# andrewcsmith/soundsym

Measured on AMD Instinct MI355X. Metric: segment-pairs/sec (DTW cost+argmin), higher is better.
Workload: dtype f32

## Files before the change

### soundsym_amd/csrc/dtw_filter.hip

```cpp
#include "ssym_internal.hpp"
#include "dtw_filter_kernel.hpp"
#include "dtw_filter_wg_kernel.hpp"
#include "dtw_filter_wg2_kernel.hpp"
#include "dtw_filter_pk_kernel.hpp"
#include "dtw_filter_sp_kernel.hpp"
#include "dtw_band_kernel.hpp"

#include <algorithm>
#include <atomic>
#include <cmath>
#include <cstdlib>

namespace ssym {

static std::atomic<unsigned long long> g_filter_wg_launches{0};
static std::atomic<unsigned long long> g_filter_wg2_launches{0};
static std::atomic<bool> g_filter_wg2{true};

int filter_pieces(int dim)
{
    static const bool k48 = ssym_knob("SSYM_FILTER_K48") != nullptr;
    return dim > kFilterMaxDim2 ? 1 : (k48 ? 2 : 3);
}

__global__ void build_filter_records_kernel(const double *__restrict__ raw, const uint64_t *__restrict__ off,
                                            const uint32_t *__restrict__ perm, uint32_t n, uint32_t dim,
                                            uint32_t dimUse, uint32_t frames_pad, int is_source,
                                            int lead, int pieces, double scale, _Float16 *__restrict__ rec,
                                            unsigned *__restrict__ resid)
{
    const uint32_t s = blockIdx.y;
    const uint32_t seg = perm[s];
    const uint32_t slot = blockIdx.x * blockDim.x + threadIdx.x;
    if (slot >= frames_pad)
        return;
    _Float16 out[kFilterRecHalfs];
#pragma unroll
    for (int i = 0; i < kFilterRecHalfs; ++i)
        out[i] = (_Float16)0.0f;
    const uint32_t nf = seg < n ? (uint32_t)(off[seg + 1] - off[seg]) : 0u;
    const uint32_t first = lead < 0 ? frames_pad - nf : (uint32_t)lead;
    const bool real = slot >= first && slot < first + nf;
    const uint32_t f = slot - first;
    const int nbase = pieces == 3 ? 28 : (pieces == 2 ? 3 : 1) * (int)dimUse;
    const int npieces = pieces == 3 ? 2 : 3;
    if (!real && is_source)
        out[filter_slot_offset(nbase)] = (_Float16)__builtin_inff();
    if (real) {
        const double *p = raw + (off[seg] + f) * dim;
        double nrm = 0.0, res2 = 0.0;
        for (uint32_t e = 0; e < dimUse; ++e) {
            const double v = p[e] * scale;
            const _Float16 h1 = (_Float16)v;
            const bool two = pieces == 2 || (pieces == 3 && (is_source || e < 2));
            const _Float16 h2 = two ? (_Float16)(v - (double)h1) : (_Float16)0.0f;
            const double vh = (double)h1 + (double)h2;
            nrm += vh * vh;
            res2 += (v - vh) * (v - vh);
            const _Float16 m1 = (_Float16)(-2.0f * (float)h1), m2 = (_Float16)(-2.0f * (float)h2);
            if (pieces == 2) {
                out[filter_slot_offset(3 * e + 0)] = is_source ? m1 : h1;
                out[filter_slot_offset(3 * e + 1)] = is_source ? m1 : h2;
                out[filter_slot_offset(3 * e + 2)] = is_source ? m2 : h1;
            } else if (pieces == 3) {
                out[filter_slot_offset(2 * e + 0)] = is_source ? m1 : h1;
                out[filter_slot_offset(2 * e + 1)] = is_source ? m2 : h1;
                if (e < 2)
                    out[filter_slot_offset(26 + e)] = is_source ? m1 : h2;
            } else {
                out[filter_slot_offset(e)] = is_source ? m1 : h1;
            }
        }
        const float r = __double2float_ru(sqrt(res2) / scale * 1.0000001);
        if (r > 0.0f)
            atomicMax(&resid[s], __float_as_uint(r));
        const _Float16 p1 = (_Float16)nrm;
        const _Float16 p2 = (_Float16)(nrm - (double)p1);
        const _Float16 p3 = (_Float16)(nrm - (double)p1 - (double)p2);
        const int mine = nbase + (is_source ? 0 : npieces), other = nbase + (is_source ? npieces : 0);
        out[filter_slot_offset(mine + 0)] = p1;
        out[filter_slot_offset(mine + 1)] = p2;
        out[filter_slot_offset(other + 0)] = (_Float16)1.0f;
        out[filter_slot_offset(other + 1)] = (_Float16)1.0f;
        if (npieces == 3) {
            out[filter_slot_offset(mine + 2)] = p3;
            out[filter_slot_offset(other + 2)] = (_Float16)1.0f;
        }
    }
    if (is_source) {
        _Float16 *dst = rec + ((size_t)s * frames_pad + slot) * kFilterRecHalfs;
#pragma unroll
        for (int i = 0; i < kFilterRecHalfs; ++i)
            dst[i] = out[i];
    } else {
#pragma unroll
        for (int h = 0; h < 2; ++h)
#pragma unroll
            for (int m = 0; m < kFilterKM; ++m) {
                _Float16 *dst = rec + tgt_rec_offset(s, frames_pad, slot, m, h);
#pragma unroll
                for (int i = 0; i < 8; ++i)
                    dst[i] = out[h * 24 + m * 8 + i];
            }
    }
}

static uint32_t band_slots(int radius, const SegmentSet &src, const SegmentSet &tgt)
{
    const uint32_t kb = (uint32_t)(2 * radius + 1 + 15) / 16 * 16;
    return std::max<uint32_t>(radius + src.max_frames, std::max<uint32_t>(tgt.max_frames, 1) + kb) + 1;
}
static size_t band_lds_bytes(int radius, const SegmentSet &src, const SegmentSet &tgt)
{
    return ((size_t)2 * band_slots(radius, src, tgt) * kFilterRecHalfs + kBandImagePad) * sizeof(_Float16);
}

bool filter_band_as_bound(const ssym_ctx *ctx, const SegmentSet &src, const SegmentSet &tgt)
{
    if (ctx->band < 0)
        return false;
    return 2 * ctx->band + 1 > 6 * 16 || band_lds_bytes(ctx->band, src, tgt) > 160 * 1024 - 64;
}

bool filter_supported(const ssym_ctx *ctx, const SegmentSet &src, const SegmentSet &tgt)
{
    if (src.light || tgt.light)
        return false;
    if (src.dim != tgt.dim)
        return false;
    if ((ctx->band < 0 || filter_band_as_bound(ctx, src, tgt)) && filter_shape((int)src.max_frames).nt == 0)
        return false;
    if (!std::isfinite(src.max_abs) || !std::isfinite(tgt.max_abs))
        return false;
    if (!std::isfinite(src.max_sqnorm_all) || !std::isfinite(tgt.max_sqnorm_all))
        return false;
    return src.n > 0 && tgt.n > 0;
}

static double common_scale(const SegmentSet &src, const SegmentSet &tgt)
{
    const double m = std::max(src.max_abs, tgt.max_abs);
    if (!(m > 0.0))
        return 1.0;
    int e = 0;
    (void)std::frexp(m, &e);
    e = std::min(std::max(6 - e, -100), 100);
    const double sq = std::max(src.max_sqnorm_all, tgt.max_sqnorm_all);
    while (e > -200 && sq * std::ldexp(1.0, 2 * e) * 1.01 >= 65000.0)
        --e;
    const double ideal = std::ldexp(1.0, e);
    if (src.rec && src.rec_scale > 0.0 && src.rec_scale <= ideal && src.rec_scale * 16.0 >= ideal)
        return src.rec_scale;
    return ideal;
}

static int32_t ensure_records(ssym_ctx *ctx, const SegmentSet &set, double scale, uint32_t slots, int lead)
{
    const size_t bytes = (size_t)set.n_pad * slots * kFilterRecHalfs * sizeof(_Float16);
    if (set.rec && set.rec_scale == scale && set.rec_bytes == bytes && set.rec_slots == slots &&
        set.rec_lead == lead)
        return SSYM_OK;
    if (set.rec && set.rec_bytes != bytes) {
        dev_free(ctx, set.rec);
        set.rec = nullptr;
    }
    if (!set.rec) {
        int32_t rca = dev_alloc(ctx, &set.rec, bytes);
        if (rca != SSYM_OK)
            return rca;
    }
    set.rec_bytes = bytes;
    dim3 grid((slots + 63) / 64, set.n_pad);
    const int dimUse = filter_dim_used((int)set.dim);
    unsigned *resid = (unsigned *)(set.max_sqnorm + 2 * (size_t)set.n_pad);
    SSYM_HIP_CHECK(ctx, hipMemsetAsync(resid, 0, sizeof(unsigned) * set.n_pad, ctx->stream));
    build_filter_records_kernel<<<grid, 64, 0, ctx->stream>>>(set.raw, set.off, set.perm, set.n, set.dim,
                                                              (uint32_t)dimUse, slots, set.is_source ? 1 : 0, lead,
                                                              filter_pieces(dimUse), scale,
                                                              (_Float16 *)set.rec, resid);
    SSYM_HIP_CHECK(ctx, hipGetLastError());
    set.rec_scale = scale;
    set.rec_slots = slots;
    set.rec_lead = lead;
    return SSYM_OK;
}

static FilterKnobs read_filter_knobs()
{
    FilterKnobs k;
    g_filter_wg2.store(true, std::memory_order_relaxed);
    if (!ssym_knob("SSYM_TEST_HOOKS"))
        return k;
    auto num = [](const char *name, int unset) {
        const char *v = ssym_knob(name);
        return v ? atoi(v) : unset;
    };
    k.pk = num("SSYM_FILTER_PK", 0) != 0;
    k.sp = num("SSYM_FILTER_SP", 1) != 0;
    const int mp = num("SSYM_SP_MULTIPAIR", 1);
    k.spMultipair = mp == 0 || mp == 2 ? mp : 1;
    k.spPairBlock = ssym_knob("SSYM_SP_PAIRBLOCK") ? std::max(num("SSYM_SP_PAIRBLOCK", 0), 0) : -1;
    k.wg = num("SSYM_FILTER_WG", k.wg) != 0;
    g_filter_wg2.store(num("SSYM_FILTER_WG2", 1) != 0, std::memory_order_relaxed);
    k.skip0 = num("SSYM_FILTER_SKIP0", 1) != 0;
    k.nt8 = ssym_knob("SSYM_FILTER_NT8") != nullptr;
    k.oneLaunch = ssym_knob("SSYM_FILTER_ONE_LAUNCH") != nullptr;
    k.longClasses = num("SSYM_FILTER_LONG_CLASSES", 1) != 0;
    k.pruneNt = num("SSYM_PRUNE_NT", 0);
    return k;
}

static const std::vector<uint32_t> &plan_lens(const SegmentSet &set, uint32_t group)
{
    if (set.plan_lens.size() != set.n_pad / group) {
        set.plan_lens.assign(set.n_pad / group, 0u);
        for (uint32_t slot = 0; slot < set.n; ++slot) {
            const uint32_t s = set.h_perm[slot];
            uint32_t &m = set.plan_lens[slot / group];
            m = std::max(m, (uint32_t)(set.h_off[s + 1] - set.h_off[s]));
        }
    }
    return set.plan_lens;
}

struct FilterCall {
    hipStream_t st;
    const SegmentSet &src, &tgt;
    bool sq;
    int ku;
    float outScale;
    float *handoff;
    unsigned *taskCtr;
    float *cmat;
    const float *abandon;
    unsigned long long *colCtr;
    const uint32_t *candSlot;
    bool wg2;
};

template <int NT, bool SQ, int KU>
static bool run_kernel(const FilterCall &c, const FilterLaunch &l)
{
    constexpr int OCC = NT == 1 ? 3 : NT == 8 ? 1 : 2;
    const dim3 grid(l.grid), block(64 * kFilterWavesPerBlock);
    const _Float16 *srec = (const _Float16 *)c.src.rec, *trec = (const _Float16 *)c.tgt.rec;
    const int rowsPad = (int)c.src.frames_pad, colsPad = (int)c.tgt.frames_pad, tgtPad = (int)c.tgt.n_pad;
    const int nSrcPairs = l.hi - l.lo, nTasks = nSrcPairs * (tgtPad / 32);
    unsigned *ctr = c.taskCtr + l.ctrSet * 8 * kTaskCtrStride;
    switch (l.kind) {
    case FilterKernel::Mp:
        if constexpr (NT == 1) {
            dtw_filter_sp_kernel<KU == 2 ? 3 : 2, SQ, 2, KU, kSpRowBlock, true><<<grid, block, 0, c.st>>>(
                srec, trec, c.src.len, c.tgt.len, rowsPad, colsPad, tgtPad, l.taskPairs, nSrcPairs, l.taskChunk, c.outScale,
                ctr, c.cmat, l.origin, l.lo, l.pairBlock);
            return true;
        }
        return false;
    case FilterKernel::Sp:
        if constexpr (NT <= 3 && (KU == 2 || NT <= 2)) {
            constexpr int OCCSP = (NT == 1 && KU == 2) ? 3 : (NT == 2 && KU == 2) ? SSYM_SP_OCC_NT2 : 2;
            dtw_filter_sp_kernel<NT, SQ, OCCSP, KU, kSpRowBlock><<<grid, block, 0, c.st>>>(
                srec, trec, c.src.len, c.tgt.len, rowsPad, colsPad, tgtPad, nSrcPairs, nTasks, l.taskChunk, c.outScale, ctr,
                c.cmat, l.origin, l.lo, l.pairBlock);
            return true;
        }
        return false;
    case FilterKernel::GenericSkip0:
        if constexpr (NT == 3 || NT == 4) {
            dtw_filter_kernel<NT, SQ, OCC, false, KU, true><<<grid, block, 0, c.st>>>(
                srec, trec, c.src.len, c.tgt.len, rowsPad, l.passes, colsPad, tgtPad, nSrcPairs, nTasks, l.taskChunk,
                c.outScale, c.handoff, ctr, c.cmat, nullptr, nullptr, nullptr, l.origin, l.lo);
            return true;
        }
        return false;
    case FilterKernel::Wg:
        if constexpr (NT == 4) {
            if (l.passes == 2 && c.wg2) {
                dtw_filter_wg2_kernel<SQ, KU><<<grid, block, 0, c.st>>>(
                    srec, trec, c.src.len, c.tgt.len, rowsPad, colsPad, tgtPad, nSrcPairs / 4, l.taskChunk, c.outScale, ctr,
                    c.cmat, l.origin, l.lo);
                g_filter_wg_launches.fetch_add(1, std::memory_order_relaxed);
                g_filter_wg2_launches.fetch_add(1, std::memory_order_relaxed);
                return true;
            }
            dtw_filter_wg_kernel<SQ, KU><<<grid, block, 0, c.st>>>(
                srec, trec, c.src.len, c.tgt.len, rowsPad, l.passes, colsPad, tgtPad, nSrcPairs / 4, l.taskChunk, c.outScale,
                c.handoff, ctr, c.cmat, l.origin, l.lo);
            g_filter_wg_launches.fetch_add(1, std::memory_order_relaxed);
            return true;
        }
        return false;
    case FilterKernel::Pk:
        if constexpr (NT == 4) {
            dtw_filter_pk_kernel<SQ, KU><<<grid, block, 0, c.st>>>(
                srec, trec, c.src.len, c.tgt.len, rowsPad, l.passes, colsPad, tgtPad, nSrcPairs, nTasks, l.taskChunk,
                c.outScale, c.handoff, ctr, c.cmat, l.origin, l.lo);
            return true;
        }
        return false;
    case FilterKernel::GenericPrune:
        dtw_filter_kernel<NT, SQ, OCC, true, KU><<<grid, block, 0, c.st>>>(
            srec, trec, c.src.len, c.tgt.len, rowsPad, l.passes, colsPad, tgtPad, nSrcPairs, nTasks, l.taskChunk, c.outScale,
            c.handoff, ctr, c.cmat, c.abandon, c.colCtr, c.candSlot, l.origin, l.lo);
        return true;
    case FilterKernel::Generic:
        dtw_filter_kernel<NT, SQ, OCC, false, KU><<<grid, block, 0, c.st>>>(
            srec, trec, c.src.len, c.tgt.len, rowsPad, l.passes, colsPad, tgtPad, nSrcPairs, nTasks, l.taskChunk, c.outScale,
            c.handoff, ctr, c.cmat, nullptr, nullptr, nullptr, l.origin, l.lo);
        return true;
    }
    return false;
}

template <int NT>
static bool run_tiles(const FilterCall &c, const FilterLaunch &l)
{
    if (c.sq)
        return c.ku == 2 ? run_kernel<NT, true, 2>(c, l) : run_kernel<NT, true, 3>(c, l);
    return c.ku == 2 ? run_kernel<NT, false, 2>(c, l) : run_kernel<NT, false, 3>(c, l);
}

static bool run_launch(const FilterCall &c, const FilterLaunch &l)
{
    switch (l.nt) {
    case 1: return run_tiles<1>(c, l);
    case 2: return run_tiles<2>(c, l);
    case 3: return run_tiles<3>(c, l);
    case 4: return run_tiles<4>(c, l);
    case 8: return run_tiles<8>(c, l);
    }
    return false;
}

template <int NTB, int WB, int OCC, bool SQ, int LASTN, bool PRUNE>
static int32_t launch_band_cfg2(ssym_ctx *ctx, const SegmentSet &src, const SegmentSet &tgt, uint32_t slots,
                                size_t lds, float outScale, float *cmat, const float *abandon,
                                unsigned long long *colCtr, const uint32_t *candSlot)
{
    const int nTgtBlocks = (int)tgt.n_pad / (32 * WB);
    const int nTasks = ((int)src.n_pad / 2) * nTgtBlocks;
    const int grid = std::max(1, std::min(ctx->num_cus, nTasks));
    int32_t rc = ensure(ctx, ctx->handoff, 8 * sizeof(unsigned));
    if (rc != SSYM_OK)
        return rc;
    unsigned *taskCtr = (unsigned *)ctx->handoff.ptr;
    rc = zero_words(ctx, taskCtr, sizeof(unsigned));
    if (rc != SSYM_OK)
        return rc;
    const bool two = filter_mfmas(filter_pieces(filter_dim_used((int)src.dim)), filter_dim_used((int)src.dim)) == 2;
    auto kern = two ? dtw_band_kernel<NTB, WB, OCC, SQ, LASTN, PRUNE, 2> : dtw_band_kernel<NTB, WB, OCC, SQ, LASTN, PRUNE, 3>;
#ifdef SSYM_BAND_PAIRCOLS_BUILD
    if constexpr (!PRUNE && LASTN == 1 && NTB >= 4 && OCC == 2) {
        const char *pc = ssym_knob("SSYM_BAND_PAIRCOLS");
        if (pc && atoi(pc) != 0)
            kern = two ? dtw_band_kernel<NTB, WB, OCC, SQ, LASTN, PRUNE, 2, true> : dtw_band_kernel<NTB, WB, OCC, SQ, LASTN, PRUNE, 3, true>;
    }
#endif
    if (lds > 64 * 1024)
        SSYM_HIP_CHECK(ctx, hipFuncSetAttribute((const void *)kern, hipFuncAttributeMaxDynamicSharedMemorySize, (int)lds));
    kern<<<dim3(grid), 64 * WB, lds, ctx->stream>>>(
        (const _Float16 *)src.rec, (const _Float16 *)tgt.rec, src.len, tgt.len, (int)slots, ctx->band,
        (int)tgt.frames_pad, (int)tgt.n_pad, nTgtBlocks, nTasks, taskCtr, outScale, cmat, abandon, colCtr, candSlot);
    SSYM_HIP_CHECK(ctx, hipGetLastError());
    return SSYM_OK;
}

template <int NTB, int WB, int OCC, bool SQ, int LASTN>
static int32_t launch_band_cfg(ssym_ctx *ctx, const SegmentSet &src, const SegmentSet &tgt, uint32_t slots,
                               size_t lds, float outScale, float *cmat, const float *abandon,
                               unsigned long long *colCtr, const uint32_t *candSlot)
{
    return abandon ? launch_band_cfg2<NTB, WB, OCC, SQ, LASTN, true>(ctx, src, tgt, slots, lds, outScale, cmat, abandon, colCtr, candSlot)
                   : launch_band_cfg2<NTB, WB, OCC, SQ, LASTN, false>(ctx, src, tgt, slots, lds, outScale, cmat, nullptr, nullptr, nullptr);
}

template <int NTB, bool SQ>
static int32_t launch_band(ssym_ctx *ctx, const SegmentSet &src, const SegmentSet &tgt, uint32_t slots,
                           size_t lds, float outScale, float *cmat, const float *abandon, unsigned long long *colCtr, const uint32_t *candSlot)
{
    const bool last1 = 2 * ctx->band + 1 == 16 * (NTB - 1) + 1;
    if constexpr (NTB <= 5)
        return last1 ? launch_band_cfg<NTB, 8, 2, SQ, 1>(ctx, src, tgt, slots, lds, outScale, cmat, abandon, colCtr, candSlot)
                     : launch_band_cfg<NTB, 8, 2, SQ, 16>(ctx, src, tgt, slots, lds, outScale, cmat, abandon, colCtr, candSlot);
    else
        return last1 ? launch_band_cfg<NTB, 4, 1, SQ, 1>(ctx, src, tgt, slots, lds, outScale, cmat, abandon, colCtr, candSlot)
                     : launch_band_cfg<NTB, 4, 1, SQ, 16>(ctx, src, tgt, slots, lds, outScale, cmat, abandon, colCtr, candSlot);
}

static int32_t launch_dtw_filter_banded(ssym_ctx *ctx, const SegmentSet &src, const SegmentSet &tgt, float *cmat,
                                        const float *abandon, unsigned long long *colCtr, const uint32_t *candSlot)
{
    if (tgt.n_pad % kBandTgtQuantum != 0 || src.n_pad % 2 != 0) {
        ctx->err = "dtw band filter: segment set not padded for the banded kernel";
        return SSYM_E_UNSUPPORTED;
    }
    const uint32_t slots = band_slots(ctx->band, src, tgt);
    const size_t lds = band_lds_bytes(ctx->band, src, tgt);
    const double scale = common_scale(src, tgt);
    int32_t rc = ensure_records(ctx, src, scale, slots, ctx->band);
    if (rc != SSYM_OK)
        return rc;
    rc = ensure_records(ctx, tgt, scale, tgt.frames_pad, 0);
    if (rc != SSYM_OK)
        return rc;
    const bool sq = ctx->squared != 0;
    const float outScale = (float)(sq ? 1.0 / (scale * scale) : 1.0 / scale);
    const int ntb = (2 * ctx->band + 1 + 15) / 16;
#define SSYM_BCASE(N_)                                                                                  \
    case N_:                                                                                            \
        return sq ? launch_band<N_, true>(ctx, src, tgt, slots, lds, outScale, cmat, abandon, colCtr, candSlot)   \
                  : launch_band<N_, false>(ctx, src, tgt, slots, lds, outScale, cmat, abandon, colCtr, candSlot);
    switch (ntb) {
        SSYM_BCASE(1) SSYM_BCASE(2) SSYM_BCASE(3) SSYM_BCASE(4) SSYM_BCASE(5) SSYM_BCASE(6)
    default:
        ctx->err = "dtw band filter: band radius too large";
        return SSYM_E_UNSUPPORTED;
    }
#undef SSYM_BCASE
}

int32_t ensure_filter_records(ssym_ctx *ctx, const SegmentSet &src, const SegmentSet &tgt, double *scale_out)
{
    const double scale = common_scale(src, tgt);
    int32_t rc = ctx->band >= 0 && !filter_band_as_bound(ctx, src, tgt)
                     ? ensure_records(ctx, src, scale, band_slots(ctx->band, src, tgt), ctx->band)
                     : ensure_records(ctx, src, scale, src.frames_pad, -1);
    if (rc == SSYM_OK)
        rc = ensure_records(ctx, tgt, scale, tgt.frames_pad, 0);
    if (scale_out)
        *scale_out = scale;
    return rc;
}

int32_t launch_dtw_filter(ssym_ctx *ctx, const SegmentSet &src, const SegmentSet &tgt, float *cmat,
                          const float *abandon, unsigned long long *colCtr, const uint32_t *candSlot)
{
    ctx->filter_launches = 1;
    if (ctx->band >= 0 && !filter_band_as_bound(ctx, src, tgt))
        return launch_dtw_filter_banded(ctx, src, tgt, cmat, abandon, colCtr, candSlot);
    const FilterShape shape = filter_shape((int)src.max_frames);
    if (shape.nt == 0 || (int)src.frames_pad != shape.rows() || src.n_pad % 8 != 0 || tgt.n_pad % 32 != 0) {
        ctx->err = "dtw filter: segment set not padded for the filter kernel";
        return SSYM_E_UNSUPPORTED;
    }
    if (((size_t)tgt.frames_pad + 3) / 4 * 1024 >= ((size_t)1 << 31)) {
        ctx->err = "dtw filter: targets too long for the hand-off rows";
        return SSYM_E_UNSUPPORTED;
    }
    const double scale = common_scale(src, tgt);
    int32_t rc = ensure_records(ctx, src, scale, src.frames_pad, -1);
    if (rc != SSYM_OK)
        return rc;
    rc = ensure_records(ctx, tgt, scale, tgt.frames_pad, 0);
    if (rc != SSYM_OK)
        return rc;
    const int gridBlocks = std::max(8, ctx->num_cus * 2 / 8 * 8);
    const size_t handBytes = (size_t)(gridBlocks / 2 * 3) * kFilterWavesPerBlock * ((tgt.frames_pad + 3) / 4) * 256 * sizeof(float);
    const size_t ctrBytes = 8 * kTaskCtrStride * sizeof(unsigned);
    rc = ensure(ctx, ctx->handoff, handBytes + kMaxClasses * ctrBytes);
    if (rc != SSYM_OK)
        return rc;
    unsigned *taskCtr = (unsigned *)((char *)ctx->handoff.ptr + handBytes);
    rc = zero_words(ctx, taskCtr, kMaxClasses * ctrBytes);
    if (rc != SSYM_OK)
        return rc;
    const bool sq = ctx->squared != 0;
    const int dimUse = filter_dim_used((int)src.dim);

    FilterPlanInput in;
    in.pairLen = plan_lens(src, 2).data(), in.groupCols = plan_lens(tgt, 32).data();
    in.srcN = src.n, in.srcNPad = src.n_pad, in.framesPad = src.frames_pad;
    in.tgtN = tgt.n, in.tgtGroups = tgt.n_pad / 32, in.tgtTotalFrames = tgt.total_frames;
    in.numCus = ctx->num_cus;
    in.ku = filter_mfmas(filter_pieces(dimUse), dimUse);
    in.abandon = abandon != nullptr;
    in.pruneSwept = ctx->prune_swept;
    in.knobs = read_filter_knobs();
    const std::vector<FilterLaunch> plan = plan_filter(in);

    ctx->filter_launches = (int)plan.size();
    ctx->launched_cells = 0;
    for (const FilterLaunch &l : plan)
        ctx->launched_cells += l.cells;
    const FilterCall call{ctx->stream, src, tgt, sq, in.ku, (float)(sq ? 1.0 / (scale * scale) : 1.0 / scale),
                          (float *)ctx->handoff.ptr, taskCtr, cmat, abandon, colCtr, candSlot,
                          g_filter_wg2.load(std::memory_order_relaxed)};
    for (const FilterLaunch &l : plan)
        if (!run_launch(call, l)) {
            ctx->err = "dtw filter: the plan names a kernel that is not built";
            return SSYM_E_UNSUPPORTED;
        }
    SSYM_HIP_CHECK(ctx, hipGetLastError());
    return SSYM_OK;
}

}

extern "C" __attribute__((visibility("default"))) unsigned long long ssym_debug_filter_wg_launches(void)
{
    return ssym::g_filter_wg_launches.load(std::memory_order_relaxed);
}

extern "C" __attribute__((visibility("default"))) unsigned long long ssym_debug_filter_wg2_launches(void)
{
    return ssym::g_filter_wg2_launches.load(std::memory_order_relaxed);
}

#ifdef SSYM_SP_PROF
extern "C" __attribute__((visibility("default"))) int ssym_debug_sp_prof(unsigned long long *out)
{
    unsigned long long zero[12] = {0, 0, 0, 0, 0, 0, 0, 0, 0, 0, 0, 0};
    if (hipMemcpyFromSymbol(out, HIP_SYMBOL(ssym::ssym_sp_prof), sizeof(zero)) != hipSuccess)
        return -1;
    return hipMemcpyToSymbol(HIP_SYMBOL(ssym::ssym_sp_prof), zero, sizeof(zero)) == hipSuccess ? 0 : -1;
}
#endif
```

### soundsym_amd/csrc/dtw_filter_wg2_kernel.hpp

```cpp
#pragma once
#include "dtw_filter_kernel.hpp"

namespace ssym {

#define SSYM_FILTER_SBASE(P_) asm volatile("" : "+s"(P_))
#define SSYM_FILTER_LANEOFF(V_) asm volatile("" : "+v"(V_))

constexpr int kFilterWg2Ring = 16;
constexpr int kFilterWg2HandBytes = 2 * 2 * 1024;
constexpr int kFilterWg2RecBytes = 2 * 16;
constexpr int kFilterWg2LenBytes = 256;
constexpr int kFilterWg2Lds = kFilterWg2Ring * kFilterSlotBytes + kFilterWg2HandBytes + kFilterWg2RecBytes + kFilterWg2LenBytes;
constexpr int wait_vmcnt_lgkm0(int n) { return wait_vmcnt(n) & ~0x0F00; }

template <bool SQ, int KU>
__global__ __launch_bounds__(64 * kFilterWavesPerBlock, 2) void dtw_filter_wg2_kernel(
    const _Float16 *__restrict__ srcRec, const _Float16 *__restrict__ tgtRec,
    const int *__restrict__ srcLen, const int *__restrict__ tgtLen, int srcRows,
    int tgtFramesPad, int mPad, int nSrcBlocks, int taskChunk, float outScale,
    unsigned *__restrict__ taskCtr, float *__restrict__ cmat, int rowOrigin, int spBase)
{
    static_assert(KU == 2 || KU == 3, "two or three operand planes per column");
    static_assert(kFilterWavesPerBlock == 4, "two pairs x two roles; a column group is one column per wave");
    constexpr int NT = 4;
    constexpr int REC = kFilterRecHalfs;
    constexpr int BR = NT * 16;
    const float INF = __builtin_inff();

    const int lane = threadIdx.x & 63;
    const int wave = __builtin_amdgcn_readfirstlane(threadIdx.x >> 6);
    const int follower = wave & 1;
    const int col = lane & 31;
    const int half = lane >> 5;
    uint32_t laneOff16 = lane * 16;
    __shared__ __attribute__((aligned(16))) char lds[kFilterWg2Lds];
    char *const ring = lds;
    char *const hand = lds + kFilterWg2Ring * kFilterSlotBytes + (wave >> 1) * 2048;
    volatile int *const record = reinterpret_cast<volatile int *>(lds + kFilterWg2Ring * kFilterSlotBytes + kFilterWg2HandBytes);

    char *const lenBuf = lds + kFilterWg2Ring * kFilterSlotBytes + kFilterWg2HandBytes + kFilterWg2RecBytes;
    uint32_t laneOff4 = lane * 4;

    const unsigned nGroups = (unsigned)mPad >> 5;

    struct Item { int tg, sp0, nCols, g; };
    Item im1{0, 0, 0, -1}, i0{0, 0, 0, -1}, i1{0, 0, 0, -1}, i2{0, 0, 0, -1};
    unsigned hop = 0;
    unsigned requests = 0;
    bool pending = false;
    bool request = false;
    unsigned tick = 0;
    unsigned feGi = 0, feEnd = 0, feHalf = 0, feXcd = 0, feRange = 0;
    bool feOn = false, feAtomic = false, feValid = false;
    unsigned feTk = 0;
    int feTg = 0, feSp0 = 0;

    auto last_group = [](const Item &it) __attribute__((always_inline)) { return 4 * (it.g + 1) >= it.nCols; };

    auto open_tick = [&](bool storeYoungest) __attribute__((always_inline)) -> bool {
        if (storeYoungest)
            __builtin_amdgcn_s_waitcnt(wait_vmcnt_lgkm0(1));
        else
            __builtin_amdgcn_s_waitcnt(wait_vmcnt_lgkm0(0));
        asm volatile("" ::: "memory");
        __builtin_amdgcn_s_barrier();
        asm volatile("" ::: "memory");
        im1 = i0;
        i0 = i1;
        i1 = i2;
        if (i2.g >= 0 && !last_group(i2)) {
            ++i2.g;
        } else if (pending) {
            const unsigned slot = (requests - 1u) & 1u;
            const int tg = __builtin_amdgcn_readfirstlane(record[4 * slot + 0]);
            const int sp0 = __builtin_amdgcn_readfirstlane(record[4 * slot + 1]);
            const int nc = __builtin_amdgcn_readfirstlane(record[4 * slot + 2]);
            if (tg >= 0) {
                i2 = Item{tg, sp0, nc, 0};
            } else {
                i2.g = -1;
                ++hop;
            }
        } else {
            i2.g = -1;
        }
        pending = false;
        if (hop >= 8u && im1.g < 0 && i0.g < 0 && i1.g < 0 && i2.g < 0)
            return false;
        request = hop < 8u && (i2.g < 0 || last_group(i2));
        if (request) {
            pending = true;
            ++requests;
        }
        feOn = request && wave == 0;
        if (feOn) {
            feXcd = (blockIdx.x + hop) & 7u;
            feRange = feXcd < nGroups ? ((nGroups - feXcd + 7u) >> 3) * (unsigned)nSrcBlocks : 0u;
            feAtomic = feGi >= feEnd;
            if (feAtomic && lane == 0)
                feTk = atomicAdd(&taskCtr[feXcd * kTaskCtrStride], (unsigned)taskChunk);
        }
        if (i2.g >= 0) {
            const int cc = max(min(4 * i2.g + wave, i2.nCols - 1), 0);
            char *slot = ring + ((4 * (tick + 2u) + (unsigned)wave) & (unsigned)(kFilterWg2Ring - 1)) * kFilterSlotBytes;
            const char *gb = reinterpret_cast<const char *>(tgtRec) +
                             ((size_t)(unsigned)i2.tg * (unsigned)tgtFramesPad + (unsigned)cc) * (kTgtFrameHalfs * 2);
            SSYM_FILTER_SBASE(gb);
            SSYM_FILTER_LANEOFF(laneOff16);
            const __attribute__((address_space(1))) void *gp =
                (const __attribute__((address_space(1))) void *)(gb + laneOff16);
            __attribute__((address_space(3))) void *lp = (__attribute__((address_space(3))) void *)slot;
            __builtin_amdgcn_global_load_lds(gp, lp, 16, 0, 0);
            __builtin_amdgcn_global_load_lds(gp, lp, 16, 1024, 0);
            if (KU == 3)
                __builtin_amdgcn_global_load_lds(gp, lp, 16, 2048, 0);
        }
        asm volatile("" ::: "memory");
        return true;
    };
    auto front_end_task = [&]() __attribute__((always_inline)) {
        if (feOn) {
            if (feAtomic) {
                feGi = (unsigned)__builtin_amdgcn_readfirstlane((int)feTk);
                feEnd = min(feGi + (unsigned)taskChunk, feRange);
                feHalf = 0;
            }
            feValid = feGi < feEnd;
            if (feValid) {
                const unsigned lin = feRange - 1u - feGi;
                feTg = (int)(feXcd + 8u * (lin / (unsigned)nSrcBlocks));
                feSp0 = spBase + 4 * (int)(lin % (unsigned)nSrcBlocks) + 2 * (int)feHalf;
                const int *gl = tgtLen + 32 * feTg;
                SSYM_FILTER_SBASE(gl);
                SSYM_FILTER_LANEOFF(laneOff4);
                __builtin_amdgcn_global_load_lds(
                    (const __attribute__((address_space(1))) void *)(reinterpret_cast<const char *>(gl) + (laneOff4 & 127u)),
                    (__attribute__((address_space(3))) void *)lenBuf, 4, 0, 0);
            }
        }
    };
    auto front_end_record = [&]() __attribute__((always_inline)) {
        if (feOn) {
            int nc = 0;
            if (feValid) {
                __builtin_amdgcn_s_waitcnt(wait_vmcnt(0));
                asm volatile("" ::: "memory");
                nc = *reinterpret_cast<volatile int *>(lenBuf + laneOff4);
#pragma unroll
                for (int o = 32; o >= 1; o >>= 1)
                    nc = max(nc, __shfl_xor(nc, o));
                nc = __builtin_amdgcn_readfirstlane(nc);
            }
            const unsigned slot = (requests - 1u) & 1u;
            if (lane == 0) {
                record[4 * slot + 0] = feValid ? feTg : -1;
                record[4 * slot + 1] = feSp0;
                record[4 * slot + 2] = nc;
            }
            if (feValid) {
                feHalf ^= 1u;
                if (feHalf == 0)
                    ++feGi;
            } else {
                feGi = feEnd = feHalf = 0;
            }
        }
    };
    auto fetch = [&](unsigned s, half8 (&B)[KU]) __attribute__((always_inline)) {
        const char *slot = ring + (s & (unsigned)(kFilterWg2Ring - 1)) * kFilterSlotBytes;
#pragma unroll
        for (int m = 0; m < KU; ++m)
            B[m] = *reinterpret_cast<const half8 *>(slot + m * 1024 + lane * 16);
    };

    half8 A[NT][KU];
    float L0[BR], L1[BR];
    half8 B0[KU], B1[KU];
    f32x16 acc;
    float prevTop = INF;
    auto start_task = [&](const Item &it, int rowBase, unsigned vg) __attribute__((always_inline)) {
        const int sp = it.sp0 + (wave >> 1);
        const int fa = srcLen[2 * sp + half];
        {
            const int arow = lane & 31;
            const int a_src = 2 * sp + ((arow >> 2) & 1);
            const int a_frm = rowBase + (arow & 3) + 4 * (arow >> 3);
            const _Float16 *abase = srcRec + ((size_t)a_src * srcRows + a_frm) * REC + half * 24;
#pragma unroll
            for (int T = 0; T < NT; ++T)
                load_rec<KU>(abase + (size_t)T * kFilterRowsPerTile * REC, A[T]);
        }
        const int r0 = srcRows - fa;
#pragma unroll
        for (int i = 0; i < BR; ++i) {
            L0[i] = (rowBase + i == r0 - 1) ? 0.0f : INF;
            L1[i] = L0[i];
        }
        prevTop = (rowBase == r0) ? 0.0f : INF;
        fetch(4u * vg, B0);
        acc = mfma_tile<KU>(A[0], B0);
    };

    if (!follower) {
        float up = INF;
        asm volatile("" : "+v"(up));
        for (;; ++tick) {
            if (!open_tick(false))
                break;
            if (i0.g >= 0) {
                const unsigned vg = tick & 3u;
                if (i0.g == 0)
                    start_task(i0, rowOrigin, vg);
                char *const handW = hand + (tick & 1u) * 1024 + lane * 4;
                auto column = [&](int q) __attribute__((always_inline)) {
                    const float diag = prevTop;
                    prevTop = up;
                    float bottom;
                    if ((q & 1) == 0) {
                        fetch(4u * vg + q + 1, B1);
                        bottom = dp_column<NT, SQ, KU>(A, B0, B1, acc, up, diag, L0, L1);
                    } else {
                        fetch(4u * vg + q + 1, B0);
                        bottom = dp_column<NT, SQ, KU>(A, B1, B0, acc, up, diag, L1, L0);
                    }
                    *reinterpret_cast<float *>(handW + q * 256) = bottom;
                };
                column(0);
                column(1);
                front_end_task();
                column(2);
                column(3);
                front_end_record();
            } else {
                front_end_task();
                front_end_record();
            }
        }
    } else {
        float res = INF;
        int fb_m1 = -1;
        bool stored = false;
        for (;; ++tick) {
            if (!open_tick(stored))
                break;
            stored = false;
            if (im1.g >= 0) {
                const unsigned vg = (tick + 3u) & 3u;
                const char *const handR = hand + ((tick + 1u) & 1u) * 1024 + lane * 4;
                float topN = *reinterpret_cast<const float *>(handR);
                if (im1.g == 0) {
                    fb_m1 = tgtLen[32 * im1.tg + col] - 1;
                    res = INF;
                    start_task(im1, rowOrigin + BR, vg);
                }
                const int j0 = 4 * im1.g;
                auto column = [&](int q) __attribute__((always_inline)) {
                    const float up = topN;
                    const float diag = prevTop;
                    prevTop = up;
                    if (q < 3)
                        topN = *reinterpret_cast<const float *>(handR + (q + 1) * 256);
                    float bottom;
                    if ((q & 1) == 0) {
                        fetch(4u * vg + q + 1, B1);
                        bottom = dp_column<NT, SQ, KU>(A, B0, B1, acc, up, diag, L0, L1);
                    } else {
                        fetch(4u * vg + q + 1, B0);
                        bottom = dp_column<NT, SQ, KU>(A, B1, B0, acc, up, diag, L1, L0);
                    }
                    res = (j0 + q == fb_m1) ? bottom : res;
                };
                column(0);
                column(1);
                column(2);
                column(3);
                if (last_group(im1)) {
                    const int sp = im1.sp0 + (wave >> 1);
                    cmat[(size_t)(2 * sp + half) * mPad + 32 * im1.tg + col] = res * outScale;
                    stored = true;
                }
            }
        }
    }
}

#undef SSYM_FILTER_SBASE
#undef SSYM_FILTER_LANEOFF

}
```

Measured before the change: 531.7 million.

## Add optional wave-role swap in wg2 filter kernel and trim follower per-column work

Adds a roles parameter that can swap which wave of each pair acts as front-end/leader, chosen by block parity or hardware wave slot, with a debug counter and optional phase-timing instrumentation. By default the swap is disabled (roles never). Separately, the kernel now records a minimum-length group index so followers pick their result once per group after the four columns instead of selecting per column (for KU==2). It also initializes only one L buffer with a ballot-guarded start row, and computes the cost store address with scalar base plus lane offset. These aim to reduce VALU work and register pressure in the follower loop, at the cost of an extra barrier and LDS word at kernel start.

```diff
diff --git a/soundsym_amd/csrc/dtw_filter.hip b/soundsym_amd/csrc/dtw_filter.hip
--- a/soundsym_amd/csrc/dtw_filter.hip
+++ b/soundsym_amd/csrc/dtw_filter.hip
@@ -16,6 +16,9 @@
 static std::atomic<unsigned long long> g_filter_wg_launches{0};
 static std::atomic<unsigned long long> g_filter_wg2_launches{0};
 static std::atomic<bool> g_filter_wg2{true};
+constexpr int kFilterWg2RolesDefault = kFilterWg2RolesNever;
+static std::atomic<int> g_filter_wg2_roles{kFilterWg2RolesDefault};
+static std::atomic<const unsigned *> g_filter_wg2_swapped{nullptr};
 
 int filter_pieces(int dim)
 {
@@ -189,6 +192,7 @@
 {
     FilterKnobs k;
     g_filter_wg2.store(true, std::memory_order_relaxed);
+    g_filter_wg2_roles.store(kFilterWg2RolesDefault, std::memory_order_relaxed);
     if (!ssym_knob("SSYM_TEST_HOOKS"))
         return k;
     auto num = [](const char *name, int unset) {
@@ -202,6 +206,9 @@
     k.spPairBlock = ssym_knob("SSYM_SP_PAIRBLOCK") ? std::max(num("SSYM_SP_PAIRBLOCK", 0), 0) : -1;
     k.wg = num("SSYM_FILTER_WG", k.wg) != 0;
     g_filter_wg2.store(num("SSYM_FILTER_WG2", 1) != 0, std::memory_order_relaxed);
+    const int roles = num("SSYM_FILTER_WG2_ROLES", kFilterWg2RolesDefault);
+    g_filter_wg2_roles.store(roles == kFilterWg2RolesNever || roles == kFilterWg2RolesOdd ? roles : kFilterWg2RolesSlot,
+                             std::memory_order_relaxed);
     k.skip0 = num("SSYM_FILTER_SKIP0", 1) != 0;
     k.nt8 = ssym_knob("SSYM_FILTER_NT8") != nullptr;
     k.oneLaunch = ssym_knob("SSYM_FILTER_ONE_LAUNCH") != nullptr;
@@ -236,6 +243,7 @@
     unsigned long long *colCtr;
     const uint32_t *candSlot;
     bool wg2;
+    int wg2Roles;
 };
 
 template <int NT, bool SQ, int KU>
@@ -278,9 +286,10 @@
             if (l.passes == 2 && c.wg2) {
                 dtw_filter_wg2_kernel<SQ, KU><<<grid, block, 0, c.st>>>(
                     srec, trec, c.src.len, c.tgt.len, rowsPad, colsPad, tgtPad, nSrcPairs / 4, l.taskChunk, c.outScale, ctr,
-                    c.cmat, l.origin, l.lo);
+                    c.cmat, l.origin, l.lo, c.wg2Roles);
                 g_filter_wg_launches.fetch_add(1, std::memory_order_relaxed);
                 g_filter_wg2_launches.fetch_add(1, std::memory_order_relaxed);
+                g_filter_wg2_swapped.store(ctr + 1, std::memory_order_relaxed);
                 return true;
             }
             dtw_filter_wg_kernel<SQ, KU><<<grid, block, 0, c.st>>>(
@@ -436,6 +445,7 @@
                           const float *abandon, unsigned long long *colCtr, const uint32_t *candSlot)
 {
     ctx->filter_launches = 1;
+    g_filter_wg2_swapped.store(nullptr, std::memory_order_relaxed);
     if (ctx->band >= 0 && !filter_band_as_bound(ctx, src, tgt))
         return launch_dtw_filter_banded(ctx, src, tgt, cmat, abandon, colCtr, candSlot);
     const FilterShape shape = filter_shape((int)src.max_frames);
@@ -484,7 +494,7 @@
         ctx->launched_cells += l.cells;
     const FilterCall call{ctx->stream, src, tgt, sq, in.ku, (float)(sq ? 1.0 / (scale * scale) : 1.0 / scale),
                           (float *)ctx->handoff.ptr, taskCtr, cmat, abandon, colCtr, candSlot,
-                          g_filter_wg2.load(std::memory_order_relaxed)};
+                          g_filter_wg2.load(std::memory_order_relaxed), g_filter_wg2_roles.load(std::memory_order_relaxed)};
     for (const FilterLaunch &l : plan)
         if (!run_launch(call, l)) {
             ctx->err = "dtw filter: the plan names a kernel that is not built";
@@ -506,6 +516,28 @@
     return ssym::g_filter_wg2_launches.load(std::memory_order_relaxed);
 }
 
+extern "C" __attribute__((visibility("default"))) long long ssym_debug_filter_wg2_swapped(void)
+{
+    const unsigned *word = ssym::g_filter_wg2_swapped.load(std::memory_order_relaxed);
+    unsigned n = 0;
+    if (!word)
+        return -1;
+    if (hipDeviceSynchronize() != hipSuccess || hipMemcpy(&n, word, sizeof(n), hipMemcpyDeviceToHost) != hipSuccess) {
+        (void)hipGetLastError();
+        return -1;
+    }
+    return (long long)n;
+}
+
+#ifdef SSYM_WG2_PHASE
+extern "C" __attribute__((visibility("default"))) int ssym_debug_wg2_phase(unsigned long long *out)
+{
+    if (hipDeviceSynchronize() != hipSuccess)
+        return -1;
+    return hipMemcpyFromSymbol(out, HIP_SYMBOL(ssym::ssym_wg2_phase), 512 * 256 * sizeof(unsigned long long)) == hipSuccess ? 0 : -1;
+}
+#endif
+
 #ifdef SSYM_SP_PROF
 extern "C" __attribute__((visibility("default"))) int ssym_debug_sp_prof(unsigned long long *out)
 {
diff --git a/soundsym_amd/csrc/dtw_filter_wg2_kernel.hpp b/soundsym_amd/csrc/dtw_filter_wg2_kernel.hpp
--- a/soundsym_amd/csrc/dtw_filter_wg2_kernel.hpp
+++ b/soundsym_amd/csrc/dtw_filter_wg2_kernel.hpp
@@ -2,6 +2,12 @@
 #include "dtw_filter_kernel.hpp"
 
 namespace ssym {
+
+constexpr int kHwIdWaveSlot = 4 | (0 << 6) | (3 << 11);
+#ifdef SSYM_WG2_PHASE
+constexpr int kHwIdAll = 4 | (0 << 6) | (31 << 11), kHwXccId = 20 | (0 << 6) | (31 << 11);
+__device__ unsigned long long ssym_wg2_phase[512][256];
+#endif
 
 #define SSYM_FILTER_SBASE(P_) asm volatile("" : "+s"(P_))
 #define SSYM_FILTER_LANEOFF(V_) asm volatile("" : "+v"(V_))
@@ -10,7 +16,9 @@
 constexpr int kFilterWg2HandBytes = 2 * 2 * 1024;
 constexpr int kFilterWg2RecBytes = 2 * 16;
 constexpr int kFilterWg2LenBytes = 256;
-constexpr int kFilterWg2Lds = kFilterWg2Ring * kFilterSlotBytes + kFilterWg2HandBytes + kFilterWg2RecBytes + kFilterWg2LenBytes;
+constexpr int kFilterWg2RoleBytes = 16;
+constexpr int kFilterWg2Lds = kFilterWg2Ring * kFilterSlotBytes + kFilterWg2HandBytes + kFilterWg2RecBytes + kFilterWg2LenBytes + kFilterWg2RoleBytes;
+constexpr int kFilterWg2RolesNever = 0, kFilterWg2RolesSlot = 1, kFilterWg2RolesOdd = 2;
 constexpr int wait_vmcnt_lgkm0(int n) { return wait_vmcnt(n) & ~0x0F00; }
 
 template <bool SQ, int KU>
@@ -18,7 +26,7 @@
     const _Float16 *__restrict__ srcRec, const _Float16 *__restrict__ tgtRec,
     const int *__restrict__ srcLen, const int *__restrict__ tgtLen, int srcRows,
     int tgtFramesPad, int mPad, int nSrcBlocks, int taskChunk, float outScale,
-    unsigned *__restrict__ taskCtr, float *__restrict__ cmat, int rowOrigin, int spBase)
+    unsigned *__restrict__ taskCtr, float *__restrict__ cmat, int rowOrigin, int spBase, int roles)
 {
     static_assert(KU == 2 || KU == 3, "two or three operand planes per column");
     static_assert(kFilterWavesPerBlock == 4, "two pairs x two roles; a column group is one column per wave");
@@ -29,7 +37,6 @@
 
     const int lane = threadIdx.x & 63;
     const int wave = __builtin_amdgcn_readfirstlane(threadIdx.x >> 6);
-    const int follower = wave & 1;
     const int col = lane & 31;
     const int half = lane >> 5;
     uint32_t laneOff16 = lane * 16;
@@ -41,10 +48,39 @@
     char *const lenBuf = lds + kFilterWg2Ring * kFilterSlotBytes + kFilterWg2HandBytes + kFilterWg2RecBytes;
     uint32_t laneOff4 = lane * 4;
 
+    volatile int *const roleWord = reinterpret_cast<volatile int *>(lenBuf + kFilterWg2LenBytes);
+    if (wave == 0) {
+        int sw = 0;
+        if (roles == kFilterWg2RolesOdd)
+            sw = (int)(blockIdx.x & 1u);
+        else if (roles == kFilterWg2RolesSlot)
+            sw = (int)(__builtin_amdgcn_s_getreg(kHwIdWaveSlot) & 1u);
+        if (lane == 0) {
+            *roleWord = sw;
+            if (sw)
+                atomicAdd(&taskCtr[1], 1u);
+        }
+    }
+    __builtin_amdgcn_s_waitcnt(wait_vmcnt_lgkm0(0));
+    asm volatile("" ::: "memory");
+    __builtin_amdgcn_s_barrier();
+    asm volatile("" ::: "memory");
+    const int swap = __builtin_amdgcn_readfirstlane(*roleWord) & 1;
+    const int follower = (wave & 1) ^ swap;
+    const int feWave = swap;
+#ifdef SSYM_WG2_PHASE
+    if (wave == 0 && lane == 0) {
+        ssym_wg2_phase[blockIdx.x & 511u][0] = (unsigned long long)__builtin_amdgcn_s_getreg(kHwIdAll) |
+                                               ((unsigned long long)__builtin_amdgcn_s_getreg(kHwXccId) << 32);
+        ssym_wg2_phase[blockIdx.x & 511u][1] = 0;
+    }
+    unsigned phaseN = 0;
+#endif
+
     const unsigned nGroups = (unsigned)mPad >> 5;
 
-    struct Item { int tg, sp0, nCols, g; };
-    Item im1{0, 0, 0, -1}, i0{0, 0, 0, -1}, i1{0, 0, 0, -1}, i2{0, 0, 0, -1};
+    struct Item { int tg, sp0, nCols, g, g0; };
+    Item im1{0, 0, 0, -1, 0}, i0{0, 0, 0, -1, 0}, i1{0, 0, 0, -1, 0}, i2{0, 0, 0, -1, 0};
     unsigned hop = 0;
     unsigned requests = 0;
     bool pending = false;
@@ -75,8 +111,9 @@
             const int tg = __builtin_amdgcn_readfirstlane(record[4 * slot + 0]);
             const int sp0 = __builtin_amdgcn_readfirstlane(record[4 * slot + 1]);
             const int nc = __builtin_amdgcn_readfirstlane(record[4 * slot + 2]);
+            const int g0 = __builtin_amdgcn_readfirstlane(record[4 * slot + 3]);
             if (tg >= 0) {
-                i2 = Item{tg, sp0, nc, 0};
+                i2 = Item{tg, sp0, nc, 0, g0};
             } else {
                 i2.g = -1;
                 ++hop;
@@ -92,7 +129,7 @@
             pending = true;
             ++requests;
         }
-        feOn = request && wave == 0;
+        feOn = request && wave == feWave;
         if (feOn) {
             feXcd = (blockIdx.x + hop) & 7u;
             feRange = feXcd < nGroups ? ((nGroups - feXcd + 7u) >> 3) * (unsigned)nSrcBlocks : 0u;
@@ -141,21 +178,26 @@
     };
     auto front_end_record = [&]() __attribute__((always_inline)) {
         if (feOn) {
-            int nc = 0;
+            int nc = 0, ncMin = 0;
             if (feValid) {
                 __builtin_amdgcn_s_waitcnt(wait_vmcnt(0));
                 asm volatile("" ::: "memory");
-                nc = *reinterpret_cast<volatile int *>(lenBuf + laneOff4);
+                nc = ncMin = *reinterpret_cast<volatile int *>(lenBuf + laneOff4);
 #pragma unroll
                 for (int o = 32; o >= 1; o >>= 1)
                     nc = max(nc, __shfl_xor(nc, o));
+#pragma unroll
+                for (int o = 16; o >= 1; o >>= 1)
+                    ncMin = min(ncMin, __shfl_xor(ncMin, o));
                 nc = __builtin_amdgcn_readfirstlane(nc);
+                ncMin = __builtin_amdgcn_readfirstlane(ncMin);
             }
             const unsigned slot = (requests - 1u) & 1u;
             if (lane == 0) {
                 record[4 * slot + 0] = feValid ? feTg : -1;
                 record[4 * slot + 1] = feSp0;
                 record[4 * slot + 2] = nc;
+                record[4 * slot + 3] = max(ncMin - 1, 0) >> 2;
             }
             if (feValid) {
                 feHalf ^= 1u;
@@ -191,12 +233,24 @@
                 load_rec<KU>(abase + (size_t)T * kFilterRowsPerTile * REC, A[T]);
         }
         const int r0 = srcRows - fa;
-#pragma unroll
-        for (int i = 0; i < BR; ++i) {
-            L0[i] = (rowBase + i == r0 - 1) ? 0.0f : INF;
-            L1[i] = L0[i];
+        const int above = r0 - 1 - rowBase;
+#pragma unroll
+        for (int i = 0; i < BR; ++i)
+            L0[i] = INF;
+        if (__builtin_amdgcn_ballot_w64((unsigned)above < (unsigned)BR) != 0) {
+            int row = above;
+            asm volatile("" : "+v"(row));
+#pragma unroll
+            for (int i = 0; i < BR; ++i)
+                L0[i] = (i == row) ? 0.0f : INF;
         }
         prevTop = (rowBase == r0) ? 0.0f : INF;
+#ifdef SSYM_WG2_PHASE
+        if (wave == 0 && lane == 0 && phaseN < 253u) {
+            ssym_wg2_phase[blockIdx.x & 511u][2 + phaseN] = __builtin_amdgcn_s_memtime();
+            ssym_wg2_phase[blockIdx.x & 511u][1] = ++phaseN;
+        }
+#endif
         fetch(4u * vg, B0);
         acc = mfma_tile<KU>(A[0], B0);
     };
@@ -254,6 +308,9 @@
                     start_task(im1, rowOrigin + BR, vg);
                 }
                 const int j0 = 4 * im1.g;
+                constexpr bool kPickBehind = KU == 2;
+                const bool picks = im1.g >= im1.g0;
+                float bq[4];
                 auto column = [&](int q) __attribute__((always_inline)) {
                     const float up = topN;
                     const float diag = prevTop;
@@ -268,15 +325,30 @@
                         fetch(4u * vg + q + 1, B0);
                         bottom = dp_column<NT, SQ, KU>(A, B1, B0, acc, up, diag, L1, L0);
                     }
-                    res = (j0 + q == fb_m1) ? bottom : res;
+                    if constexpr (kPickBehind)
+                        bq[q] = bottom;
+                    else
+                        res = (j0 + q == fb_m1) ? bottom : res;
                 };
                 column(0);
                 column(1);
                 column(2);
                 column(3);
+                if (kPickBehind && picks) {
+                    asm volatile("" : "+v"(res));
+#pragma unroll
+                    for (int q = 0; q < 4; ++q)
+                        res = (j0 + q == fb_m1) ? bq[q] : res;
+                }
                 if (last_group(im1)) {
                     const int sp = im1.sp0 + (wave >> 1);
-                    cmat[(size_t)(2 * sp + half) * mPad + 32 * im1.tg + col] = res * outScale;
+                    char *cb = reinterpret_cast<char *>(cmat + ((size_t)(2 * sp) * mPad + 32 * im1.tg));
+                    SSYM_FILTER_SBASE(cb);
+                    SSYM_FILTER_LANEOFF(laneOff4);
+                    const uint32_t laneCost = (laneOff4 & 127u) + (laneOff4 >> 7) * ((uint32_t)mPad * 4u);
+                    float r = res;
+                    asm volatile("" : "+v"(r));
+                    *reinterpret_cast<float *>(cb + laneCost) = r * outScale;
                     stored = true;
                 }
             }
```

Result: no change. 536.0 million (median of 6 runs) (+0.8%).
